# wenet-e2e/wenet

Hardware: AMD Instinct MI355X
Metric: audio-seconds/sec (RTF^-1), 12L Conformer fbank80, ctc_prefix_beam_search (higher is better)
Workload: dtype f32 (feed-forward and subsampling-conv2 GEMMs: fp32 operands as three exact bf16 planes, six plane products on the bf16 matrix cores, f32 accumulate -- error <= the v_mfma_f32 kernel's, tests/test_gpu_x6.py; everything else v_mfma_f32)

## Files before the change

include/wenet_amd.h:

```cpp
#ifndef WENET_AMD_H_
#define WENET_AMD_H_

#include <stdint.h>

#ifdef __cplusplus
extern "C" {
#endif

typedef struct wn_model wn_model;

typedef struct {
  int32_t feat_dim;
  int32_t d_model;
  int32_t n_heads;
  int32_t ffn_dim;
  int32_t n_layers;
  int32_t cnn_kernel;
  int32_t causal;
  int32_t use_dynamic_chunk;
  int32_t static_chunk_size;
  int32_t vocab;
  int32_t has_cmvn;
  int32_t dec_heads;
  int32_t dec_ffn_dim;
// ... 180 lines not shown
                    int32_t K, float alpha, int32_t act, void* stream);
int wn_op_gemm_skinny(const float* A_dev, const float* W_dev, const float* bias_dev,
                      const float* resid_dev, float* C_dev, int32_t M, int32_t N, int32_t K,
                      int32_t act, int32_t w_bf16, int32_t split_k, void* stream);
int wn_op_gemm_bf16_stored(const float* A_dev, const float* W_dev, const float* bias_dev,
                           const float* resid_dev, void* C_dev, int32_t M, int32_t N,
                           int32_t K, float alpha, int32_t act, int32_t c_bf16,
                           void* stream);
int wn_op_gemm_lowp(const void* A_dev, const void* W_dev, const void* a_scale_dev,
                    const void* w_scale_dev, const float* bias_dev,
                    const float* resid_dev, void* C_dev, void* c_scale_dev, int32_t M,
                    int32_t N, int32_t K, float alpha, int32_t act, int32_t c_mode,
                    int32_t dtype, void* stream);
int wn_op_mx_quantize(const float* x_dev, int32_t rows, int32_t K, void* q_dev,
                      void* scale_dev, void* stream);
int wn_op_ffn_fused(const float* X_dev, const float* W1_dev, const float* b1_dev,
                    const float* W2_dev, const float* b2_dev, float* x_inout_dev,
                    const float* ln_w_dev, const float* ln_b_dev, float* y_out_dev,
                    int32_t M, int32_t D, int32_t F, int32_t act, float alpha, float eps,
                    void* stream);
int wn_op_gemm_x6(const float* A_dev, const float* W_dev, const float* bias_dev,
                  const float* resid_dev, float* C_dev, int32_t M, int32_t N, int32_t K,
                  float alpha, int32_t act, int32_t bm, int32_t reps, void* stream);
int wn_op_ffn_x6(const float* X_dev, const float* W1_dev, const float* b1_dev,
                 const float* W2_dev, const float* b2_dev, float* x_inout_dev,
                 const float* ln_w_dev, const float* ln_b_dev, float* y_out_dev, int32_t M,
                 int32_t D, int32_t F, int32_t act, float alpha, float eps, int32_t reps,
                 void* stream);
int wn_op_gemm_x6r(const float* A_dev, const float* W_dev, const float* bias_dev,
                   float* x_inout_dev, const float* ln_w_dev, const float* ln_b_dev,
                   float* y_dev, float* C_dev, int32_t M, int32_t N, int32_t epi, float alpha,
                   float eps, int32_t reps, void* stream);

int wn_op_gemm_x6r512(const float* A, const float* W, const float* bias, float* x_inout,
                      const float* ln_w, const float* ln_b, float* y, const float* W2,
                      const float* bias2, float* C, int32_t M, int32_t N, int32_t epi, float alpha,
                      float eps, int32_t reps, void* stream);
int wn_op_log_add(const double* a_dev, const double* b_dev, double* out_dev,
                  int32_t n, void* stream);
int wn_op_layernorm(const float* x_dev, const float* w_dev, const float* b_dev,
                    float* y_dev, int32_t M, int32_t D, float eps, void* stream);

typedef struct wn_attention_op {
  const void* Q; const void* K; const void* V;
  int32_t ldq, ldk, ldv;
  int32_t q_rows, kv_rows;
  const float* P; int32_t ldp, p_rows;
  const int32_t* p_off;
  const float* bias_u; const float* bias_v;
  void* O; int32_t ldo;
  const int32_t* q_off; const int32_t* q_len;
  const int32_t* kv_off; const int32_t* kv_len;
  int32_t n_seq, n_heads;
  int32_t mask_mode, chunk_size, left_chunks;
  float scale;
  int32_t flags;
  int32_t precision;
  int32_t x6_galign;
} wn_attention_op;
#define WN_ATTN_FOLD 1
#define WN_ATTN_PREFOLD 2
#define WN_ATTN_QKV_BF16 4
#define WN_ATTN_O_BF16 8
int wn_op_attention(const wn_attention_op* op, int32_t* form_out, void* stream);
int wn_op_dwconv(const float* x, int32_t ldx, const float* wt, const float* bias,
                 const float* cpad, const float* ln_w, const float* ln_b, int32_t norm_mode,
// ... 58 lines not shown
```

wenet_amd/_lib.py:

```python
import ctypes
import os
from ctypes import (POINTER, Structure, c_char_p, c_double, c_float, c_int32,
                    c_int64, c_void_p)

_HERE = os.path.dirname(os.path.abspath(__file__))
LIB_PATH = os.path.join(_HERE, 'libwenet_amd.so')


class WnConfig(Structure):
    _fields_ = [(n, c_int32) for n in (
        'feat_dim', 'd_model', 'n_heads', 'ffn_dim', 'n_layers', 'cnn_kernel',
        'causal', 'use_dynamic_chunk', 'static_chunk_size', 'vocab',
        'has_cmvn', 'dec_heads', 'dec_ffn_dim', 'dec_layers', 'dec_r_layers',
        'bidirectional', 'sos', 'eos', 'max_pos')] + [('norm_eps', c_float)] + [
            (n, c_int32) for n in ('encoder_type', 'input_layer', 'activation',
                                   'key_bias', 'cnn_norm',
                                   'dec_activation', 'dec_key_bias', 'dec_src_key_bias',
                                   'dec_learned_pos', 'dec_max_pos')]


class WnTransducerConfig(Structure):
    _fields_ = [(n, c_int32) for n in ('pred_embed', 'pred_hidden', 'pred_layers', 'pred_out',
                                       'join_dim', 'blank')]


class WnTensor(Structure):
    _fields_ = [('name', c_char_p), ('data', POINTER(c_float)),
                ('numel', c_int64)]


class WnStreamResult(Structure):
    _fields_ = [('n_hyps', POINTER(c_int32)), ('hyp_lens', POINTER(c_int32)),
                ('hyp_tlens', POINTER(c_int32)), ('hyp_tokens', POINTER(c_int32)),
                ('hyp_times', POINTER(c_int32)), ('hyp_scores', POINTER(c_double)),
                ('hyp_viterbi', POINTER(c_double)), ('frames_decoded', POINTER(c_int32)),
                ('trailing_blank', POINTER(c_int32)), ('max_len', c_int32)]


class WnAttentionOp(Structure):
    _fields_ = [('Q', c_void_p), ('K', c_void_p), ('V', c_void_p),
                ('ldq', c_int32), ('ldk', c_int32), ('ldv', c_int32),
                ('q_rows', c_int32), ('kv_rows', c_int32),
                ('P', c_void_p), ('ldp', c_int32), ('p_rows', c_int32),
                ('p_off', POINTER(c_int32)), ('bias_u', c_void_p), ('bias_v', c_void_p),
                ('O', c_void_p), ('ldo', c_int32),
                ('q_off', POINTER(c_int32)), ('q_len', POINTER(c_int32)),
                ('kv_off', POINTER(c_int32)), ('kv_len', POINTER(c_int32)),
                ('n_seq', c_int32), ('n_heads', c_int32), ('mask_mode', c_int32),
                ('chunk_size', c_int32), ('left_chunks', c_int32), ('scale', c_float),
                ('flags', c_int32), ('precision', c_int32), ('x6_galign', c_int32)]


EXPORTS = [
    'wn_last_error', 'wn_version', 'wn_model_create', 'wn_model_destroy', 'wn_model_clone',
    'wn_model_set_precision', 'wn_model_get_precision', 'wn_batch_size', 'wn_model_set_encode_gate', 'wn_op_gemm_bf16',
    'wn_op_gemm_bf16_stored',
    'wn_attention_beam_search', 'wn_attention_beam_search_prompt', 'wn_attention_truncated',
    'wn_op_gemm_skinny', 'wn_encode_chunk_batch', 'wn_op_gemm_lowp', 'wn_op_mx_quantize', 'wn_op_ffn_fused', 'wn_op_gemm_x6', 'wn_op_ffn_x6', 'wn_op_gemm_x6r', 'wn_op_gemm_x6r512', 'wn_profile_kernel_name', 'wn_profile_ffn_split', 'wn_profile_ffn_clocks', 'wn_profile_gemm_clocks', 'wn_filter_blank_embedding',
    'wn_workspace_create', 'wn_resample_length', 'wn_resample', 'wn_fbank', 'wn_log_mel', 'wn_encode', 'wn_encode_chunk', 'wn_set_encoder_out',
    'wn_ctc_logprobs', 'wn_set_ctc_probs', 'wn_ctc_greedy_search', 'wn_ctc_force_align',
    'wn_set_context_graph', 'wn_ctc_prefix_beam_search', 'wn_attention_rescoring', 'wn_rescore', 'wn_rescore_prefetch', 'wn_decoder_forward', 'wn_decoder_next_topk', 'wn_op_gemm',
    'wn_op_layernorm', 'wn_op_log_add', 'wn_op_attention', 'wn_op_dwconv', 'wn_op_conv1',
    'wn_op_ctc_rows', 'wn_debug_set', 'wn_profile_enable',
    'wn_profile_collect', 'wn_tune_set', 'wn_model_tune_set', 'wn_tune_get',
    'wn_stream_create', 'wn_stream_destroy', 'wn_stream_set_endpoint', 'wn_stream_reset',
    'wn_stream_advance', 'wn_stream_advance_encoded',
    'wn_model_create_transducer', 'wn_transducer_greedy_search', 'wn_op_lstm_step',
    'wn_op_joint_argmax',
]

_lib = None


def lib():
    global _lib
    if _lib is not None:
        return _lib
    if not os.path.exists(LIB_PATH):
        raise RuntimeError(
            f'{LIB_PATH} is missing: build it with `python -m wenet_amd.build` '
            '(hipcc --offload-arch=gfx950). wenet_amd has no CPU fallback.')
    import torch
    L = ctypes.CDLL(LIB_PATH, mode=ctypes.RTLD_GLOBAL)
    i32, i64, f32, vp = c_int32, c_int64, c_float, c_void_p
    pi32, pf64 = POINTER(c_int32), POINTER(c_double)
    L.wn_last_error.restype = c_char_p
    L.wn_profile_kernel_name.restype = c_char_p
    L.wn_profile_kernel_name.argtypes = [vp]
    L.wn_profile_ffn_split.restype = c_int32
    L.wn_profile_ffn_split.argtypes = [vp]
    L.wn_profile_ffn_clocks.argtypes = [POINTER(ctypes.c_uint64)]
# ... 29 lines not shown
    L.wn_stream_create.argtypes = [vp, i32, i32, i32, i32, POINTER(vp), vp]
    L.wn_stream_destroy.argtypes = [vp]
    L.wn_stream_set_endpoint.argtypes = [vp, f32, f32]
    L.wn_stream_reset.argtypes = [vp, i32, pi32, vp]
    L.wn_stream_advance.argtypes = [vp, i32, pi32, vp, pi32, i32, i32, i32,
                                    POINTER(WnStreamResult), vp]
    L.wn_stream_advance_encoded.argtypes = [vp, i32, pi32, vp, pi32, i32, i32,
                                            POINTER(WnStreamResult), vp]
    L.wn_attention_rescoring.argtypes = [vp, i32, pi32, pi32, pi32, i32, f32,
                                         POINTER(f32), POINTER(f32), vp]
    L.wn_rescore.argtypes = [vp, i32, pi32, pi32, pi32, pf64, i32, c_double, c_double, pi32,
                             POINTER(f32), pf64, pf64, POINTER(f32), vp]
    L.wn_rescore_prefetch.argtypes = [vp, i32, vp]
    L.wn_decoder_forward.argtypes = [vp, i32, i32, i32, pi32, pi32, i32, vp, vp]
    L.wn_decoder_next_topk.argtypes = [vp, i32, pi32, pi32, pi32, i32, i32,
                                       POINTER(f32), pi32, vp]
    L.wn_attention_beam_search.argtypes = [vp, i32, i32, f32, pi32, pi32, vp]
    L.wn_attention_beam_search_prompt.argtypes = [vp, i32, i32, f32, pi32, i32, pi32, pi32, vp]
    L.wn_attention_truncated.argtypes = [vp]
    L.wn_op_gemm.argtypes = [vp, vp, vp, vp, vp, i32, i32, i32, f32, i32, vp]
    L.wn_op_gemm_skinny.argtypes = [vp, vp, vp, vp, vp, i32, i32, i32, i32, i32, i32, vp]
    L.wn_op_gemm_bf16.argtypes = L.wn_op_gemm.argtypes
    L.wn_op_gemm_bf16_stored.argtypes = [vp, vp, vp, vp, vp, i32, i32, i32, f32, i32, i32, vp]
    L.wn_op_gemm_lowp.argtypes = [vp, vp, vp, vp, vp, vp, vp, vp, i32, i32, i32, f32, i32, i32,
                                  i32, vp]
    L.wn_op_mx_quantize.argtypes = [vp, i32, i32, vp, vp, vp]
    L.wn_op_ffn_fused.argtypes = [vp, vp, vp, vp, vp, vp, vp, vp, vp, i32, i32, i32, i32, f32,
                                  f32, vp]
    L.wn_op_gemm_x6.argtypes = [vp, vp, vp, vp, vp, i32, i32, i32, f32, i32, i32, i32, vp]
    L.wn_op_ffn_x6.argtypes = [vp, vp, vp, vp, vp, vp, vp, vp, vp, i32, i32, i32, i32, f32,
                               f32, i32, vp]
    L.wn_filter_blank_embedding.argtypes = [vp, vp, pi32, pi32, vp]
    L.wn_op_gemm_x6r.argtypes = [vp, vp, vp, vp, vp, vp, vp, vp, i32, i32, i32, f32, f32, i32, vp]
    L.wn_op_gemm_x6r512.argtypes = [vp, vp, vp, vp, vp, vp, vp, vp, vp, vp, i32, i32, i32, f32, f32,
                                    i32, vp]
    L.wn_model_set_precision.argtypes = [vp, i32]
    L.wn_model_get_precision.argtypes = [vp]
    L.wn_batch_size.argtypes = [vp]
    L.wn_batch_size.restype = i32
    L.wn_model_set_encode_gate.argtypes = [vp, vp]
    L.wn_op_layernorm.argtypes = [vp, vp, vp, vp, i32, i32, f32, vp]
    L.wn_op_log_add.argtypes = [vp, vp, vp, i32, vp]
    L.wn_op_attention.argtypes = [POINTER(WnAttentionOp), pi32, vp]
    L.wn_op_dwconv.argtypes = [vp, i32, vp, vp, vp, vp, vp, i32, vp, i32, pi32, pi32, i32, i32,
                               i32, i32, i32, i32, f32, vp]
    L.wn_op_conv1.argtypes = [vp, vp, vp, vp, vp, vp, pi32, pi32, i32, i32, i32, i32, i32, i32,
                              vp]
    L.wn_op_ctc_rows.argtypes = [vp, i32, i32, i32, i32, i32, f32, vp, vp, vp, i32, vp]
    L.wn_debug_set.argtypes = [vp, c_char_p, i32]
    L.wn_tune_set.argtypes = [c_char_p, i32]
    L.wn_model_tune_set.argtypes = [vp, c_char_p, i32]
    L.wn_tune_get.argtypes = [vp, c_char_p, pi32]
    L.wn_profile_enable.argtypes = [vp, i32]
    L.wn_profile_collect.argtypes = [vp, pi32, pf64, pf64]
    L.wn_model_create_transducer.argtypes = [POINTER(WnConfig), POINTER(WnTransducerConfig),
                                             POINTER(WnTensor), i32, i32, POINTER(vp)]
    L.wn_transducer_greedy_search.argtypes = [vp, i32, pi32, pi32, i32, pi32, vp]
    L.wn_op_lstm_step.argtypes = [vp, POINTER(vp), i32, vp, vp, vp, vp, vp, vp, i32, i32, i32,
                                  i32, vp]
    L.wn_op_joint_argmax.argtypes = [vp, i32, vp, i32, pi32, pi32, vp, vp, i32, i32, i32, pi32,
                                     POINTER(f32), vp]
    for n in EXPORTS:
        if n not in ('wn_last_error', 'wn_version', 'wn_model_destroy',
                     'wn_resample_length', 'wn_profile_kernel_name',
                     'wn_profile_ffn_split'):
            getattr(L, n).restype = i32
# ... 29 lines not shown
```

wenet_amd/csrc/cabi_ops.hip:

```cpp
#include "model_state.h"
#include "x6.h"

namespace wn {
namespace {

__global__ __launch_bounds__(256) void conv1_image_unpack_kernel(
    const char* __restrict__ img, int tiles, const int* __restrict__ t1_off,
    const int* __restrict__ t1_len, int F1, int C, float* __restrict__ out) {
  const int b = blockIdx.y;
  const int n = t1_len[b] * F1 * (C / 8);
  const int ne = (F1 + 1) / 2;
  for (int i = blockIdx.x * 256 + threadIdx.x; i < n; i += gridDim.x * 256) {
    const int cg = i % (C / 8), px = i / (C / 8);
    const int fr = px / F1, pos = px - fr * F1;
    const int f1 = pos < ne ? 2 * pos : 2 * (pos - ne) + 1;
    const int row = (t1_off[b] + fr) * F1;
    const char* src = img + x3_piece(cg >> 1, tiles, row + pos, cg & 1);
    const bf16x8 p0 = *reinterpret_cast<const bf16x8*>(src);
    const bf16x8 p1 = *reinterpret_cast<const bf16x8*>(src + X3_REC);
    const bf16x8 p2 = *reinterpret_cast<const bf16x8*>(src + 2 * X3_REC);
    float* o = out + ((int64_t)row + f1) * C + cg * 8;
#pragma unroll
    for (int e = 0; e < 8; ++e) o[e] = ((float)p0[e] + (float)p1[e]) + (float)p2[e];
  }
// ... 210 lines not shown
      g1.A = X; g1.lda = D; g1.a_bytes = (int64_t)M * D * 4;
      g1.epi = 0; g1.C = hf.as<float>(); g1.ldc = F;
      g2.A = hf.as<float>(); g2.lda = F; g2.a_bytes = (int64_t)M * F * 4;
    } else {
      WN_TRY(x6_split(X, M, D, D, x3.as<char>(), s));
      g1.A3 = x3.as<char>(); g1.epi = 2; g1.C3 = h3.as<char>();
      g2.A3 = h3.as<char>();
    }
    WN_TRY(gemm_x6(g1, s));
    WN_TRY(gemm_x6(g2, s));
    if (r + 1 < reps) continue;
    WN_TRY(ffn_reduce_ln(x, part.as<float>(), S, b2, alpha, ln_w, ln_b, nullptr, nullptr, y,
                         M, D, eps, 0, s));
  }
  return 0;
}

int wn_op_gemm_x6r(const float* A, const float* W, const float* bias, float* x_inout,
                   const float* ln_w, const float* ln_b, float* y, float* C, int32_t M,
                   int32_t N, int32_t epi, float alpha, float eps, int32_t reps, void* stream) {
  WN_CHECK(A && W && M > 0 && gemm_x6r_supported(M, N, 256, epi), "gemm_x6r: shape");
  hipStream_t s = (hipStream_t)stream;
  static thread_local DevBuf w3;
  WN_TRY(w3.ensure(x6_bytes(N, 256)));
  WN_TRY(x6_split(W, N, 256, 256, w3.as<char>(), s));
  X6RArgs a;
  a.A = A; a.lda = 256; a.W3 = w3.as<char>(); a.bias = bias; a.M = M; a.N = N; a.epi = epi;
  a.C = C; a.ldc = N; a.resid = x_inout; a.ldr = N; a.alpha = alpha; a.x_out = x_inout;
  a.ldx = N; a.ln_w = ln_w; a.ln_b = ln_b; a.eps = eps; a.y = y; a.ldy = N;
  for (int r = 0; r < (reps > 0 ? reps : 1); ++r) WN_TRY(gemm_x6r(a, s));
  return 0;
}

int wn_op_gemm_x6r512(const float* A, const float* W, const float* bias, float* x_inout,
                      const float* ln_w, const float* ln_b, float* y, const float* W2,
                      const float* bias2, float* C, int32_t M, int32_t N, int32_t epi, float alpha,
                      float eps, int32_t reps, void* stream) {
  WN_CHECK(A && W && M > 0 && gemm_x6r512_supported(M, N, epi), "gemm_x6r512: shape");
  WN_CHECK(epi != 3 || (W2 && C), "gemm_x6r512: the chained epilogue needs W2 and C");
  hipStream_t s = (hipStream_t)stream;
  static thread_local DevBuf w3, w3b;
  WN_TRY(w3.ensure(x6_bytes(N, 512)));
  WN_TRY(x6_split(W, N, 512, 512, w3.as<char>(), s));
  X6RArgs a;
  a.A = A; a.lda = 512; a.K = 512; a.W3 = w3.as<char>(); a.bias = bias; a.M = M; a.N = N;
  a.epi = epi; a.C = C; a.ldc = epi == 3 ? 512 : N; a.resid = x_inout; a.ldr = N; a.alpha = alpha;
  a.x_out = x_inout; a.ldx = N; a.ln_w = ln_w; a.ln_b = ln_b; a.eps = eps; a.y = y; a.ldy = N;
  if (epi == 3) {
    WN_TRY(w3b.ensure(x6_bytes(1024, 512)));
    WN_TRY(x6_split(W2, 1024, 512, 512, w3b.as<char>(), s));
    a.W3b = w3b.as<char>(); a.bias2 = bias2;
  }
  for (int r = 0; r < (reps > 0 ? reps : 1); ++r) WN_TRY(gemm_x6r(a, s));
  return 0;
}

int wn_op_log_add(const double* a_dev, const double* b_dev, double* out_dev,
                  int32_t n, void* stream) {
  return log_add_pairs(a_dev, b_dev, out_dev, n, (hipStream_t)stream);
}

int wn_op_layernorm(const float* x, const float* w, const float* b, float* y,
                    int32_t M, int32_t D, float eps, void* stream) {
  return layernorm(x, D, w, b, y, D, M, D, eps, (hipStream_t)stream);
}

// ... 197 lines not shown
```

wenet_amd/csrc/gemm_x6r.hip:

```cpp
#include "common.h"
#include "kernels.h"
#include "rowregs.h"
#include "attn_x6_img.h"
#include "x6.h"

namespace wn {

namespace {

#define WAVE_LDS_ORDER() asm volatile("s_waitcnt lgkmcnt(0)" ::: "memory")

constexpr int RK = 256;
constexpr int RKB = RK / 16;

__device__ unsigned long long g_x6r_clk[8][8];
template <int NT, int EPI, int PF, int PRO = 0>
__global__ __launch_bounds__(256, 1) void x6r_kernel(X6RArgs p) {
  const bool stamp = blockIdx.x == gridDim.x / 2 && threadIdx.x == 0;
  unsigned long long k0 = __builtin_readcyclecounter(), k1 = 0, k2 = 0, k3 = 0, k4 = 0, kp = 0;
  const unsigned long long rt0 = __builtin_amdgcn_s_memrealtime();
  __shared__ float red[2][4][32];
  constexpr int PATCH = 4 * 32 * (NT * 128 + 16) > 32 * 1040 ? 4 * 32 * (NT * 128 + 16) : 32 * 1040;
  __shared__ __attribute__((aligned(16))) char patch[PATCH];
  __shared__ __attribute__((aligned(16))) char ximg[RKB * 3 * 1024];
  const int tid = threadIdx.x, lane = tid & 63;
  const int wave = __builtin_amdgcn_readfirstlane(tid >> 6);
  __builtin_assume(wave >= 0 && wave < 4);
  const int hi = lane >> 5, li = lane & 31;
  const int m0 = blockIdx.x * 32;
  const int row = m0 + li;
  const int rowc = min(row, p.M - 1);

  {
    f32x4 rowv[8];
    if constexpr (PRO == 1) {
      const int c = lane * 4;
      const f32x4 b2 = *reinterpret_cast<const f32x4*>(p.pro_b2 + c);
      f32x4 acc8[8], xo8[8];
      int r8[8];
#pragma unroll
      for (int j = 0; j < 8; ++j) {
        r8[j] = min(m0 + wave * 8 + j, p.M - 1);
        acc8[j] = b2;
        xo8[j] = *reinterpret_cast<const f32x4*>(p.pro_x + (int64_t)r8[j] * RK + c);
      }
      int sl = 0;
      for (; sl + 4 <= p.pro_S; sl += 4) {
        f32x4 v[4][8];
#pragma unroll
        for (int u = 0; u < 4; ++u)
#pragma unroll
          for (int j = 0; j < 8; ++j)
            v[u][j] = *reinterpret_cast<const f32x4*>(
                p.pro_P + ((int64_t)(sl + u) * p.M + r8[j]) * RK + c);
#pragma unroll
        for (int u = 0; u < 4; ++u)
#pragma unroll
// ... 151 lines not shown
        bb.load(a.ln_b, lane);
#pragma unroll
        for (int r = 0; r < R; ++r) {
          const float var = sq[r] * (1.0f / RK);
          const float rstd = 1.0f / sqrtf(var + a.eps);
#pragma unroll
          for (int e = 0; e < 4; ++e)
            acc[r].v[e] = (acc[r].v[e] - sm[r]) * rstd * ww.v[e] + bb.v[e];
        }
      } else {
        RowRegs<4> sc, sh;
        sc.load(a.ln_w, lane);
        sh.load(a.ln_b, lane);
#pragma unroll
        for (int r = 0; r < R; ++r)
#pragma unroll
          for (int e = 0; e < 4; ++e) acc[r].v[e] = fmaf(acc[r].v[e], sc.v[e], sh.v[e]);
      }
#pragma unroll
      for (int r = 0; r < R; ++r)
#pragma unroll
        for (int e = 0; e < 4; ++e) rowv[r][e] = on[r] ? silu_f(acc[r].v[e]) : 0.f;
    } else {
#pragma unroll
      for (int j = 0; j < 8; ++j) {
        const int r = min(m0 + wave * 8 + j, p.M - 1);
        rowv[j] = *reinterpret_cast<const f32x4*>(p.A + (int64_t)r * p.lda + lane * 4);
      }
    }
    asm volatile("" : "+v"(rowv[0]), "+v"(rowv[7]));
    kp = __builtin_readcyclecounter();
#pragma unroll
    for (int j = 0; j < 8; ++j)
      *reinterpret_cast<f32x4*>(patch + (wave * 8 + j) * 1040 + lane * 16) = rowv[j];
  }
  const int Tn = (p.N + 31) >> 5;
  const char* wb = reinterpret_cast<const char*>(p.W3) + ((int64_t)wave * NT * 3) * X3_REC +
                   lane * 16;
  const int64_t kstride = (int64_t)Tn * X3_TILE;
  bf16x8 wf[PF + 1][NT][3];
  auto load_w = [&](int ks) {
    const char* q = wb + ks * kstride;
#pragma unroll
    for (int t = 0; t < NT; ++t)
#pragma unroll
      for (int pl = 0; pl < 3; ++pl)
        wf[ks % (PF + 1)][t][pl] = *reinterpret_cast<const bf16x8*>(q + (t * 3 + pl) * X3_REC);
  };
  constexpr bool RELOAD = PF == 1;
  auto load_rec = [&](int ks, int t, int pl) {
    wf[ks % (PF + 1)][t][pl] =
        *reinterpret_cast<const bf16x8*>(wb + ks * kstride + (t * 3 + pl) * X3_REC);
  };
  __builtin_amdgcn_sched_barrier(0);
#pragma unroll
  for (int s = 0; s < (RELOAD ? 2 : PF); ++s) load_w(s);
  __syncthreads();
  k1 = __builtin_readcyclecounter();
  auto split_quarter = [&]() {
#pragma unroll
    for (int j = 0; j < RKB / 4; ++j) {
      const int ks = wave * (RKB / 4) + j;
      const f32x4 a4 = *reinterpret_cast<const f32x4*>(patch + li * 1040 + ks * 64 + hi * 32);
      const f32x4 b4 = *reinterpret_cast<const f32x4*>(patch + li * 1040 + ks * 64 + hi * 32 + 16);
      bf16x8 x3[3];
#pragma unroll
      for (int e = 0; e < 4; ++e) {
        const Split3 sa = split3(a4[e]), sb = split3(b4[e]);
        x3[0][e] = sa.h0; x3[1][e] = sa.h1; x3[2][e] = sa.h2;
        x3[0][4 + e] = sb.h0; x3[1][4 + e] = sb.h1; x3[2][4 + e] = sb.h2;
      }
#pragma unroll
      for (int pl = 0; pl < 3; ++pl)
        *reinterpret_cast<bf16x8*>(ximg + (ks * 3 + pl) * 1024 + lane * 16) = x3[pl];
    }
  };
  bf16x8 xf[2][3];
  auto load_x = [&](int ks) {
#pragma unroll
    for (int pl = 0; pl < 3; ++pl)
      xf[ks & 1][pl] = *reinterpret_cast<const bf16x8*>(ximg + (ks * 3 + pl) * 1024 + lane * 16);
  };
  split_quarter();
  __syncthreads();
  load_x(0);

  f32x16 acc[NT];
#pragma unroll
  for (int t = 0; t < NT; ++t)
#pragma unroll
    for (int r = 0; r < 16; ++r) acc[t][r] = 0.f;
  const int ecol = wave * NT * 32 + 4 * hi;
  f32x4 ebias[NT][4], elw[(EPI == 1 || EPI == 3) ? NT : 1][4], elb[(EPI == 1 || EPI == 3) ? NT : 1][4];
#pragma unroll
  for (int t = 0; t < NT; ++t)
#pragma unroll
    for (int g = 0; g < 4; ++g) {
// ... 5 lines not shown
        elb[t][g] = *reinterpret_cast<const f32x4*>(p.ln_b + c);
      }
    }
  k2 = __builtin_readcyclecounter();

  constexpr int PW[6] = {2, 0, 1, 1, 0, 0}, PX[6] = {0, 2, 1, 0, 1, 0};
#pragma unroll
  for (int ks = 0; ks < RKB; ++ks) {
    if (!RELOAD && ks + PF < RKB) load_w(ks + PF);
    if (ks + 1 < RKB) load_x(ks + 1);
#pragma unroll
    for (int q = 0; q < 6; ++q) {
#pragma unroll
      for (int t = 0; t < NT; ++t)
        acc[t] = __builtin_amdgcn_mfma_f32_32x32x16_bf16(wf[ks % (PF + 1)][t][PW[q]],
                                                         xf[ks & 1][PX[q]], acc[t], 0, 0, 0);
      if (RELOAD && ks + 2 < RKB && (q == 0 || q == 3 || q == 5)) {
        __builtin_amdgcn_sched_barrier(0);
#pragma unroll
        for (int t = 0; t < NT; ++t) load_rec(ks + 2, t, q == 0 ? 2 : q == 3 ? 1 : 0);
      }
    }
    __builtin_amdgcn_sched_barrier(0);
  }

  asm volatile("" : "+v"(acc[0]), "+v"(acc[NT - 1]));
  k3 = __builtin_readcyclecounter();
  const int col0 = wave * NT * 32;
  constexpr int SEG = NT * 128;
  constexpr int PST = SEG + 16;
  constexpr int LPR = SEG / 16;
  constexpr int NIT = 32 * LPR / 64;
  __syncthreads();
  char* wp = patch + wave * (32 * PST);
  auto put = [&](const f32x4 (&v)[NT][4]) {
#pragma unroll
    for (int t = 0; t < NT; ++t)
#pragma unroll
      for (int g = 0; g < 4; ++g)
        *reinterpret_cast<f32x4*>(wp + li * PST + (t * 32 + 8 * g + 4 * hi) * 4) = v[t][g];
  };
  auto get = [&](f32x4 (&v)[NT][4]) {
#pragma unroll
    for (int t = 0; t < NT; ++t)
#pragma unroll
      for (int g = 0; g < 4; ++g)
        v[t][g] = *reinterpret_cast<const f32x4*>(wp + li * PST + (t * 32 + 8 * g + 4 * hi) * 4);
  };
  auto store_rows = [&](float* base, int ld) {
#pragma unroll
    for (int it = 0; it < NIT; ++it) {
      const int q = it * 64 + lane, r = q / LPR, pc = q - r * LPR;
      const f32x4 v = *reinterpret_cast<const f32x4*>(wp + r * PST + pc * 16);
      if (m0 + r < p.M && col0 + pc * 4 < p.N)
        *reinterpret_cast<f32x4*>(base + (int64_t)(m0 + r) * ld + col0 + pc * 4) = v;
    }
  };
  if constexpr (EPI == 0) {
    f32x4 v[NT][4];
#pragma unroll
    for (int t = 0; t < NT; ++t)
#pragma unroll
      for (int g = 0; g < 4; ++g) {
        v[t][g] = f32x4{acc[t][4 * g], acc[t][4 * g + 1], acc[t][4 * g + 2], acc[t][4 * g + 3]} +
                  ebias[t][g];
      }
    put(v);
// ... 172 lines not shown
        }
    s2 += __shfl_xor(s2, 32, 64);
    if (hi == 0) red[1][wave][li] = s2;
    __syncthreads();
    const float var =
        ((red[1][0][li] + red[1][1][li]) + (red[1][2][li] + red[1][3][li])) / (float)p.N;
    const float rstd = 1.0f / sqrtf(var + p.eps);
#pragma unroll
    for (int t = 0; t < NT; ++t)
#pragma unroll
      for (int g = 0; g < 4; ++g) {
        const f32x4 w = elw[t][g], b = elb[t][g];
#pragma unroll
        for (int e = 0; e < 4; ++e) v[t][g][e] = (v[t][g][e] - mean) * rstd * w[e] + b[e];
      }
    if (p.y != nullptr) {
      put(v);
      store_rows(p.y, p.ldy);
    }
    if constexpr (EPI == 1) {
      if (p.y3 != nullptr) {
        const int tiles_m = (p.M + 31) >> 5;
#pragma unroll
        for (int t = 0; t < NT; ++t)
          x3_store_tile(v[t], p.y3, (col0 + t * 32) >> 4, tiles_m, blockIdx.x, hi, li);
      }
    }
    if constexpr (EPI == 3) {
      __syncthreads();
#pragma unroll
      for (int t = 0; t < NT; ++t)
#pragma unroll
        for (int g = 0; g < 4; ++g)
          *reinterpret_cast<f32x4*>(patch + li * 1040 + (col0 + t * 32 + 8 * g + 4 * hi) * 4) =
              v[t][g];
      constexpr int NT2 = 4, PF2 = 2;
      const char* wb2 = reinterpret_cast<const char*>(p.W3b) +
                        ((int64_t)wave * NT2 * 3) * X3_REC + lane * 16;
      const int64_t kstride2 = (int64_t)16 * X3_TILE;
      bf16x8 wf2[PF2 + 1][NT2][3];
      auto load_w2 = [&](int ks) {
        const char* q = wb2 + ks * kstride2;
#pragma unroll
        for (int t = 0; t < NT2; ++t)
#pragma unroll
          for (int pl = 0; pl < 3; ++pl)
            wf2[ks % (PF2 + 1)][t][pl] =
                *reinterpret_cast<const bf16x8*>(q + (t * 3 + pl) * X3_REC);
      };
#pragma unroll
      for (int s2i = 0; s2i < PF2; ++s2i) load_w2(s2i);
      __syncthreads();
      split_quarter();
      __syncthreads();
      load_x(0);
      f32x16 acc2[NT2];
#pragma unroll
      for (int t = 0; t < NT2; ++t)
#pragma unroll
        for (int r = 0; r < 16; ++r) acc2[t][r] = 0.f;
      f32x4 ebias2[NT2][4];
#pragma unroll
      for (int t = 0; t < NT2; ++t)
#pragma unroll
        for (int g = 0; g < 4; ++g) {
          ebias2[t][g] = f32x4{0.f, 0.f, 0.f, 0.f};
          if (p.bias2)
            ebias2[t][g] = *reinterpret_cast<const f32x4*>(p.bias2 + wave * NT2 * 32 + t * 32 +
                                                           8 * g + 4 * hi);
        }
#pragma unroll
      for (int ks = 0; ks < RKB; ++ks) {
        if (ks + PF2 < RKB) load_w2(ks + PF2);
        if (ks + 1 < RKB) load_x(ks + 1);
#pragma unroll
        for (int q = 0; q < 6; ++q)
#pragma unroll
          for (int t = 0; t < NT2; ++t)
            acc2[t] = __builtin_amdgcn_mfma_f32_32x32x16_bf16(wf2[ks % (PF2 + 1)][t][PW[q]],
                                                              xf[ks & 1][PX[q]], acc2[t], 0, 0, 0);
        __builtin_amdgcn_sched_barrier(0);
      }
      __syncthreads();
      const int c2 = wave * NT2 * 32;
      char* wp2 = patch + wave * (32 * 272);
#pragma unroll
      for (int u = 0; u < 2; ++u)
#pragma unroll
        for (int g = 0; g < 4; ++g) {
          const int c = c2 + 2 * u * 32 + 8 * g + 4 * hi;
          f32x4 a = f32x4{acc2[2 * u][4 * g], acc2[2 * u][4 * g + 1], acc2[2 * u][4 * g + 2],
                          acc2[2 * u][4 * g + 3]};
          f32x4 gt = f32x4{acc2[2 * u + 1][4 * g], acc2[2 * u + 1][4 * g + 1],
                           acc2[2 * u + 1][4 * g + 2], acc2[2 * u + 1][4 * g + 3]};
          a += ebias2[2 * u][g];
          gt += ebias2[2 * u + 1][g];
          f32x4 o;
#pragma unroll
          for (int e = 0; e < 4; ++e) o[e] = a[e] * wn_rcp(1.0f + wn_exp(-gt[e]));
          *reinterpret_cast<f32x4*>(wp2 + li * 272 + (u * 32 + 8 * g + 4 * hi) * 4) = o;
        }
#pragma unroll
      for (int it = 0; it < 8; ++it) {
        const int q = it * 64 + lane, r = q >> 4, pc = q & 15;
        const f32x4 o = *reinterpret_cast<const f32x4*>(wp2 + r * 272 + pc * 16);
        if (m0 + r < p.M)
          *reinterpret_cast<f32x4*>(p.C + (int64_t)(m0 + r) * p.ldc + c2 / 2 + pc * 4) = o;
      }
    }
  }
  asm volatile("s_waitcnt vmcnt(0)" ::: "memory");
  k4 = __builtin_readcyclecounter();
  if (stamp) {
    unsigned long long* o = g_x6r_clk[(EPI == 4 ? 0 : EPI) + (PRO != 0 ? 4 : 0)];
    o[0] = k0; o[1] = k1; o[2] = k2; o[3] = k3; o[4] = k4; o[5] = kp;
    o[6] = rt0; o[7] = __builtin_amdgcn_s_memrealtime();
  }
}

template <int NT, int EPI, int PF, int PRO = 0>
int launch_x6r(const X6RArgs& a, hipStream_t s) {
  hipLaunchKernelGGL((x6r_kernel<NT, EPI, PF, PRO>), dim3(cdiv(a.M, 32)), dim3(256), 0, s, a);
  WN_HIP(hipGetLastError());
  return 0;
}

}

int gemm_x6r_clocks(unsigned long long* out) {
  WN_HIP(hipDeviceSynchronize());
  WN_HIP(hipMemcpyFromSymbol(out, HIP_SYMBOL(g_x6r_clk), sizeof(g_x6r_clk)));
  return 0;
}

bool gemm_x6r_supported(int M, int N, int K, int epi) {
  if (K == 512) return gemm_x6r512_supported(M, N, epi);
  if (K != RK || M <= 0) return false;
  if (epi == 1 || epi == 3) return N == 256;
  if (epi == 2) return N == 512;
  if (epi == 4) return N == 768;
  return N == 256 || N == 512 || N == 768;
}

int gemm_x6r(const X6RArgs& a, hipStream_t s) {
  if (a.K == 512) return gemm_x6r512(a, s);
  WN_CHECK(a.K == RK, "gemm_x6r: K must be 256 or 512");
  if (a.pro_P) {
    WN_CHECK((a.epi == 0 || a.epi == 4) && a.N == 768 && a.W3 && a.M > 0 && a.pro_S >= 1 &&
                 a.pro_b2 && a.pro_x && a.ln_w && a.ln_b && a.C && a.ldc % 4 == 0,
             "gemm_x6r: prologue fold arguments");
    if (a.epi == 4) {
      WN_CHECK(a.at_img && a.at_P && a.at_ldp % 4 == 0 && a.at_u && a.at_v && a.at_row_utt &&
                   a.at_off && a.bias, "gemm_x6r: key-tile image arguments (epi 4)");
      return launch_x6r<6, 4, 1, 1>(a, s);
    }
    return launch_x6r<6, 0, 1, 1>(a, s);
  }
  WN_CHECK((a.A || a.dw_on) && a.W3 && a.lda % 4 == 0 && a.epi != 4 &&
               gemm_x6r_supported(a.M, a.N, RK, a.epi), "gemm_x6r: shape");
  if (a.dw_on) {
    WN_CHECK(a.epi == 1 && a.N == 256 && a.W3 && a.M > 0 && a.dw.D == 256 && a.dw.M == a.M &&
                 a.dw.x && a.dw.ldx % 4 == 0 && a.dw.wt && a.dw.bias && a.dw.cpad && a.dw.ln_w &&
                 a.dw.ln_b && a.dw.row_utt && a.dw.off && a.dw.len && a.dw.K >= 1 &&
                 a.resid && a.x_out && a.ln_w && a.ln_b && (a.y || a.y3) && a.ldr % 4 == 0 &&
                 a.ldx % 4 == 0 && a.ldy % 4 == 0, "gemm_x6r: depthwise-conv prologue arguments");
    return launch_x6r<2, 1, 3, 2>(a, s);
  }
  if (a.epi == 1) {
    WN_CHECK(a.resid && a.x_out && a.ln_w && a.ln_b && (a.y || a.y3) && a.ldr % 4 == 0 && a.ldx % 4 == 0 &&
                 a.ldy % 4 == 0, "gemm_x6r: row-LN epilogue arguments");
    return launch_x6r<2, 1, 3>(a, s);
  }
  if (a.epi == 3) {
    WN_CHECK(a.resid && a.x_out && a.ln_w && a.ln_b && a.ldr % 4 == 0 && a.ldx % 4 == 0 &&
                 (a.y == nullptr || a.ldy % 4 == 0) && a.W3b && a.C && a.ldc % 4 == 0,
             "gemm_x6r: chained row-LN + GLU arguments");
    return launch_x6r<2, 3, 3>(a, s);
  }
  WN_CHECK(a.C && a.ldc % 4 == 0, "gemm_x6r: no output");
  if (a.epi == 2) return launch_x6r<4, 2, 2>(a, s);
  switch (a.N) {
    case 256: return launch_x6r<2, 0, 3>(a, s);
    case 512: return launch_x6r<4, 0, 2>(a, s);
    default: return launch_x6r<6, 0, 1>(a, s);
  }
}

}
```

wenet_amd/csrc/tune.h:

```cpp
#pragma once
#include <stdint.h>

#include <string>

namespace wn {

#define WN_TUNE_KEYS(X)                                                                         \
                          \
  X(gemm_tile_bf16, 0)                                                                          \
                            \
  X(bf16_store, 1)                                                                              \
                      \
  X(lp_probe, 0)                                                                                \
                       \
  X(attn_split, 0)                                                                              \
                     \
  X(attn_bf16, 1)                                                                               \
                 \
  X(attn_bf16_nw, 0)                                                                            \
                                                                            \
  X(attn_bf16_defer, 80)                                                                        \
                                                              \
  X(attn_bf16_dma, 1)                                                                           \
                        \
  X(qkv_bf16, 1)                                                                                \
            \
  X(fp8_min_tiles, 192)                                                                         \
       \
  X(ffn_fused, 1)                                                                               \
                                                                   \
  X(gemm_x6, 1)                                                                                 \
                                         \
  X(x6_linear, 1)                                                                               \
                      \
  X(x6_af32, 0)                                                                                 \
            \
  X(x6_conv_af32, 0)                                                                            \
     \
  X(enc_gate_pos, 0)                                                                            \
                                                            \
  X(x6_conv_bm, 128)                                                                            \
                    \
  X(x6_probe, 0)                                                                                \
                     \
  X(ffn_x6f, 1)                                                                                 \
            \
  X(ffn_ximg, 1)                                                                                \
                             \
  X(ffn_x6f_ring, 3)                                                                            \
                  \
  X(ffn_x6f_var, 0)                                                                             \
                                                                        \
  X(x6r, 1)                                                                                     \
                  \
  X(x6r_chain, 1)                                                                               \
          \
  X(x6r_dwc, 1)                                                                                 \
        \
  X(x6r_pro, 1)                                                                                 \
            \
  X(x6r512_rows, 0)                                                                             \
                 \
  X(gemm_rowln, 1)                                                                              \
          \
  X(dwconv_tiled, 1)                                                                            \
                               \
  X(attn_x6, 1)                                                                                 \
                   \
  X(attn_xcd, 1)                                                                                \
        \
  X(attn_x6_galign, 2)                                                                          \
                             \
  X(attn_x6_order, 1)                                                                           \
    \
  X(attn_x6_var, 0)                                                                             \
        \
  X(attn_fold, 1)                                                                               \
                  \
  X(rescore_groups, 1)                                                                          \
                                                \
  X(rescore_prefetch, 1)                                                                        \
    \
  X(beam_weak_hash, 0)                                                                          \
                                                                              \
  X(beam_lds_pool, 1)                                                                           \
    \
  X(sync_spin, 1)                                                                               \
                         \
  X(ctc_wave, 1)                                                                                \
        \
// ... 23 lines not shown
```

Measured before the change: 72300.

## Fit two x6r blocks per CU by reusing the activation-image LDS for patches

For the NT=2 x6r GEMM variants, the separate patch scratch buffer is removed and its staging is carved into quarters of the ximg LDS buffer. This lets launch bounds request two blocks per CU, raising occupancy to hide memory latency. The split loads are read into registers before being overwritten, and the second GEMM's bias load is deferred into the last K iterations. A tune key (x6r_pair=0) restores single-block occupancy via dynamic LDS padding. It also adds a test entry point, wn_op_gemm_x6r_chain.

```diff
diff --git a/include/wenet_amd.h b/include/wenet_amd.h
--- a/include/wenet_amd.h
+++ b/include/wenet_amd.h
@@ -236,6 +236,11 @@
                    float* y_dev, float* C_dev, int32_t M, int32_t N, int32_t epi, float alpha,
                    float eps, int32_t reps, void* stream);
 
+int wn_op_gemm_x6r_chain(const float* A, const float* W, const float* bias, float* x_inout,
+                         const float* ln_w, const float* ln_b, float* y, const float* W2,
+                         const float* bias2, float* C, int32_t M, float alpha, float eps,
+                         void* stream);
+
 int wn_op_gemm_x6r512(const float* A, const float* W, const float* bias, float* x_inout,
                       const float* ln_w, const float* ln_b, float* y, const float* W2,
                       const float* bias2, float* C, int32_t M, int32_t N, int32_t epi, float alpha,
diff --git a/wenet_amd/_lib.py b/wenet_amd/_lib.py
--- a/wenet_amd/_lib.py
+++ b/wenet_amd/_lib.py
@@ -56,7 +56,7 @@
     'wn_model_set_precision', 'wn_model_get_precision', 'wn_batch_size', 'wn_model_set_encode_gate', 'wn_op_gemm_bf16',
     'wn_op_gemm_bf16_stored',
     'wn_attention_beam_search', 'wn_attention_beam_search_prompt', 'wn_attention_truncated',
-    'wn_op_gemm_skinny', 'wn_encode_chunk_batch', 'wn_op_gemm_lowp', 'wn_op_mx_quantize', 'wn_op_ffn_fused', 'wn_op_gemm_x6', 'wn_op_ffn_x6', 'wn_op_gemm_x6r', 'wn_op_gemm_x6r512', 'wn_profile_kernel_name', 'wn_profile_ffn_split', 'wn_profile_ffn_clocks', 'wn_profile_gemm_clocks', 'wn_filter_blank_embedding',
+    'wn_op_gemm_skinny', 'wn_encode_chunk_batch', 'wn_op_gemm_lowp', 'wn_op_mx_quantize', 'wn_op_ffn_fused', 'wn_op_gemm_x6', 'wn_op_ffn_x6', 'wn_op_gemm_x6r', 'wn_op_gemm_x6r_chain', 'wn_op_gemm_x6r512', 'wn_profile_kernel_name', 'wn_profile_ffn_split', 'wn_profile_ffn_clocks', 'wn_profile_gemm_clocks', 'wn_filter_blank_embedding',
     'wn_workspace_create', 'wn_resample_length', 'wn_resample', 'wn_fbank', 'wn_log_mel', 'wn_encode', 'wn_encode_chunk', 'wn_set_encoder_out',
     'wn_ctc_logprobs', 'wn_set_ctc_probs', 'wn_ctc_greedy_search', 'wn_ctc_force_align',
     'wn_set_context_graph', 'wn_ctc_prefix_beam_search', 'wn_attention_rescoring', 'wn_rescore', 'wn_rescore_prefetch', 'wn_decoder_forward', 'wn_decoder_next_topk', 'wn_op_gemm',
@@ -152,6 +152,7 @@
                                f32, i32, vp]
     L.wn_filter_blank_embedding.argtypes = [vp, vp, pi32, pi32, vp]
     L.wn_op_gemm_x6r.argtypes = [vp, vp, vp, vp, vp, vp, vp, vp, i32, i32, i32, f32, f32, i32, vp]
+    L.wn_op_gemm_x6r_chain.argtypes = [vp, vp, vp, vp, vp, vp, vp, vp, vp, vp, i32, f32, f32, vp]
     L.wn_op_gemm_x6r512.argtypes = [vp, vp, vp, vp, vp, vp, vp, vp, vp, vp, i32, i32, i32, f32, f32,
                                     i32, vp]
     L.wn_model_set_precision.argtypes = [vp, i32]
diff --git a/wenet_amd/csrc/cabi_ops.hip b/wenet_amd/csrc/cabi_ops.hip
--- a/wenet_amd/csrc/cabi_ops.hip
+++ b/wenet_amd/csrc/cabi_ops.hip
@@ -266,6 +266,25 @@
   return 0;
 }
 
+int wn_op_gemm_x6r_chain(const float* A, const float* W, const float* bias, float* x_inout,
+                         const float* ln_w, const float* ln_b, float* y, const float* W2,
+                         const float* bias2, float* C, int32_t M, float alpha, float eps,
+                         void* stream) {
+  WN_CHECK(A && W && W2 && C && M > 0 && gemm_x6r_supported(M, 256, 256, 3), "gemm_x6r: shape");
+  hipStream_t s = (hipStream_t)stream;
+  static thread_local DevBuf w3, w3b;
+  WN_TRY(w3.ensure(x6_bytes(256, 256)));
+  WN_TRY(x6_split(W, 256, 256, 256, w3.as<char>(), s));
+  WN_TRY(w3b.ensure(x6_bytes(512, 256)));
+  WN_TRY(x6_split(W2, 512, 256, 256, w3b.as<char>(), s));
+  X6RArgs a;
+  a.A = A; a.lda = 256; a.W3 = w3.as<char>(); a.bias = bias; a.M = M; a.N = 256; a.epi = 3;
+  a.C = C; a.ldc = 256; a.resid = x_inout; a.ldr = 256; a.alpha = alpha; a.x_out = x_inout;
+  a.ldx = 256; a.ln_w = ln_w; a.ln_b = ln_b; a.eps = eps; a.y = y; a.ldy = 256;
+  a.W3b = w3b.as<char>(); a.bias2 = bias2;
+  return gemm_x6r(a, s);
+}
+
 int wn_op_gemm_x6r512(const float* A, const float* W, const float* bias, float* x_inout,
                       const float* ln_w, const float* ln_b, float* y, const float* W2,
                       const float* bias2, float* C, int32_t M, int32_t N, int32_t epi, float alpha,
diff --git a/wenet_amd/csrc/gemm_x6r.hip b/wenet_amd/csrc/gemm_x6r.hip
--- a/wenet_amd/csrc/gemm_x6r.hip
+++ b/wenet_amd/csrc/gemm_x6r.hip
@@ -15,14 +15,20 @@
 
 __device__ unsigned long long g_x6r_clk[8][8];
 template <int NT, int EPI, int PF, int PRO = 0>
-__global__ __launch_bounds__(256, 1) void x6r_kernel(X6RArgs p) {
+__global__ __launch_bounds__(256, NT == 2 ? 2 : 1) void x6r_kernel(X6RArgs p) {
   const bool stamp = blockIdx.x == gridDim.x / 2 && threadIdx.x == 0;
   unsigned long long k0 = __builtin_readcyclecounter(), k1 = 0, k2 = 0, k3 = 0, k4 = 0, kp = 0;
   const unsigned long long rt0 = __builtin_amdgcn_s_memrealtime();
   __shared__ float red[2][4][32];
-  constexpr int PATCH = 4 * 32 * (NT * 128 + 16) > 32 * 1040 ? 4 * 32 * (NT * 128 + 16) : 32 * 1040;
+  constexpr bool PAIR = NT == 2;
+  constexpr int QUART = (RKB / 4) * 3 * 1024;
+  constexpr int QST = 272;
+  constexpr int PATCH = PAIR ? 16 :
+      4 * 32 * (NT * 128 + 16) > 32 * 1040 ? 4 * 32 * (NT * 128 + 16) : 32 * 1040;
   __shared__ __attribute__((aligned(16))) char patch[PATCH];
   __shared__ __attribute__((aligned(16))) char ximg[RKB * 3 * 1024];
+  static_assert(!PAIR || sizeof(red) + sizeof(ximg) <= 163840 / 2 - 1280, "NT = 2: LDS of two blocks per CU");
+  static_assert(!PAIR || (32 * QST <= QUART && NT * 128 + 16 == QST), "NT = 2: the patches fit their quarter");
   const int tid = threadIdx.x, lane = tid & 63;
   const int wave = __builtin_amdgcn_readfirstlane(tid >> 6);
   __builtin_assume(wave >= 0 && wave < 4);
@@ -240,7 +246,11 @@
     kp = __builtin_readcyclecounter();
 #pragma unroll
     for (int j = 0; j < 8; ++j)
-      *reinterpret_cast<f32x4*>(patch + (wave * 8 + j) * 1040 + lane * 16) = rowv[j];
+      if constexpr (PAIR)
+        *reinterpret_cast<f32x4*>(ximg + (lane >> 4) * QUART + (wave * 8 + j) * QST +
+                                  (lane & 15) * 16) = rowv[j];
+      else
+        *reinterpret_cast<f32x4*>(patch + (wave * 8 + j) * 1040 + lane * 16) = rowv[j];
   }
   const int Tn = (p.N + 31) >> 5;
   const char* wb = reinterpret_cast<const char*>(p.W3) + ((int64_t)wave * NT * 3) * X3_REC +
@@ -266,11 +276,27 @@
   __syncthreads();
   k1 = __builtin_readcyclecounter();
   auto split_quarter = [&]() {
+    f32x4 qa[PAIR ? RKB / 4 : 1], qb[PAIR ? RKB / 4 : 1];
+    if constexpr (PAIR) {
+      const char* qp = ximg + wave * QUART + li * QST + hi * 32;
+#pragma unroll
+      for (int j = 0; j < RKB / 4; ++j) {
+        qa[j] = *reinterpret_cast<const f32x4*>(qp + j * 64);
+        qb[j] = *reinterpret_cast<const f32x4*>(qp + j * 64 + 16);
+      }
+      WAVE_LDS_ORDER();
+    }
 #pragma unroll
     for (int j = 0; j < RKB / 4; ++j) {
       const int ks = wave * (RKB / 4) + j;
-      const f32x4 a4 = *reinterpret_cast<const f32x4*>(patch + li * 1040 + ks * 64 + hi * 32);
-      const f32x4 b4 = *reinterpret_cast<const f32x4*>(patch + li * 1040 + ks * 64 + hi * 32 + 16);
+      f32x4 a4, b4;
+      if constexpr (PAIR) {
+        a4 = qa[j];
+        b4 = qb[j];
+      } else {
+        a4 = *reinterpret_cast<const f32x4*>(patch + li * 1040 + ks * 64 + hi * 32);
+        b4 = *reinterpret_cast<const f32x4*>(patch + li * 1040 + ks * 64 + hi * 32 + 16);
+      }
       bf16x8 x3[3];
 #pragma unroll
       for (int e = 0; e < 4; ++e) {
@@ -342,7 +368,7 @@
   constexpr int LPR = SEG / 16;
   constexpr int NIT = 32 * LPR / 64;
   __syncthreads();
-  char* wp = patch + wave * (32 * PST);
+  char* wp = PAIR ? ximg + wave * QUART : patch + wave * (32 * PST);
   auto put = [&](const f32x4 (&v)[NT][4]) {
 #pragma unroll
     for (int t = 0; t < NT; ++t)
@@ -581,8 +607,11 @@
       for (int t = 0; t < NT; ++t)
 #pragma unroll
         for (int g = 0; g < 4; ++g)
-          *reinterpret_cast<f32x4*>(patch + li * 1040 + (col0 + t * 32 + 8 * g + 4 * hi) * 4) =
-              v[t][g];
+          if constexpr (PAIR)
+            *reinterpret_cast<f32x4*>(wp + li * QST + (t * 32 + 8 * g + 4 * hi) * 4) = v[t][g];
+          else
+            *reinterpret_cast<f32x4*>(patch + li * 1040 + (col0 + t * 32 + 8 * g + 4 * hi) * 4) =
+                v[t][g];
       constexpr int NT2 = 4, PF2 = 2;
       const char* wb2 = reinterpret_cast<const char*>(p.W3b) +
                         ((int64_t)wave * NT2 * 3) * X3_REC + lane * 16;
@@ -609,19 +638,23 @@
 #pragma unroll
         for (int r = 0; r < 16; ++r) acc2[t][r] = 0.f;
       f32x4 ebias2[NT2][4];
-#pragma unroll
-      for (int t = 0; t < NT2; ++t)
-#pragma unroll
-        for (int g = 0; g < 4; ++g) {
-          ebias2[t][g] = f32x4{0.f, 0.f, 0.f, 0.f};
-          if (p.bias2)
-            ebias2[t][g] = *reinterpret_cast<const f32x4*>(p.bias2 + wave * NT2 * 32 + t * 32 +
-                                                           8 * g + 4 * hi);
-        }
+      auto load_bias2 = [&](int t0) {
+#pragma unroll
+        for (int t = t0; t < t0 + NT2 / 2; ++t)
+#pragma unroll
+          for (int g = 0; g < 4; ++g) {
+            ebias2[t][g] = f32x4{0.f, 0.f, 0.f, 0.f};
+            if (p.bias2)
+              ebias2[t][g] = *reinterpret_cast<const f32x4*>(p.bias2 + wave * NT2 * 32 + t * 32 +
+                                                             8 * g + 4 * hi);
+          }
+      };
 #pragma unroll
       for (int ks = 0; ks < RKB; ++ks) {
         if (ks + PF2 < RKB) load_w2(ks + PF2);
         if (ks + 1 < RKB) load_x(ks + 1);
+        if (ks == RKB - 2) load_bias2(0);
+        if (ks == RKB - 1) load_bias2(NT2 / 2);
 #pragma unroll
         for (int q = 0; q < 6; ++q)
 #pragma unroll
@@ -632,7 +665,7 @@
       }
       __syncthreads();
       const int c2 = wave * NT2 * 32;
-      char* wp2 = patch + wave * (32 * 272);
+      char* wp2 = PAIR ? wp : patch + wave * (32 * 272);
 #pragma unroll
       for (int u = 0; u < 2; ++u)
 #pragma unroll
@@ -668,8 +701,11 @@
 }
 
 template <int NT, int EPI, int PF, int PRO = 0>
-int launch_x6r(const X6RArgs& a, hipStream_t s) {
-  hipLaunchKernelGGL((x6r_kernel<NT, EPI, PF, PRO>), dim3(cdiv(a.M, 32)), dim3(256), 0, s, a);
+int launch_x6r(const X6RArgs& a, hipStream_t s, bool alone = false) {
+  constexpr int LDS_ALONE = 32 * 1024;
+  const int dyn = NT == 2 && alone ? LDS_ALONE : 0;
+  if (dyn) WN_MAX_DYN_LDS((x6r_kernel<NT, EPI, PF, PRO>), LDS_ALONE);
+  hipLaunchKernelGGL((x6r_kernel<NT, EPI, PF, PRO>), dim3(cdiv(a.M, 32)), dim3(256), dyn, s, a);
   WN_HIP(hipGetLastError());
   return 0;
 }
@@ -707,29 +743,30 @@
   }
   WN_CHECK((a.A || a.dw_on) && a.W3 && a.lda % 4 == 0 && a.epi != 4 &&
                gemm_x6r_supported(a.M, a.N, RK, a.epi), "gemm_x6r: shape");
+  const bool alone = tune().x6r_pair == 0;
   if (a.dw_on) {
     WN_CHECK(a.epi == 1 && a.N == 256 && a.W3 && a.M > 0 && a.dw.D == 256 && a.dw.M == a.M &&
                  a.dw.x && a.dw.ldx % 4 == 0 && a.dw.wt && a.dw.bias && a.dw.cpad && a.dw.ln_w &&
                  a.dw.ln_b && a.dw.row_utt && a.dw.off && a.dw.len && a.dw.K >= 1 &&
                  a.resid && a.x_out && a.ln_w && a.ln_b && (a.y || a.y3) && a.ldr % 4 == 0 &&
                  a.ldx % 4 == 0 && a.ldy % 4 == 0, "gemm_x6r: depthwise-conv prologue arguments");
-    return launch_x6r<2, 1, 3, 2>(a, s);
+    return launch_x6r<2, 1, 3, 2>(a, s, alone);
   }
   if (a.epi == 1) {
     WN_CHECK(a.resid && a.x_out && a.ln_w && a.ln_b && (a.y || a.y3) && a.ldr % 4 == 0 && a.ldx % 4 == 0 &&
                  a.ldy % 4 == 0, "gemm_x6r: row-LN epilogue arguments");
-    return launch_x6r<2, 1, 3>(a, s);
+    return launch_x6r<2, 1, 3>(a, s, alone);
   }
   if (a.epi == 3) {
     WN_CHECK(a.resid && a.x_out && a.ln_w && a.ln_b && a.ldr % 4 == 0 && a.ldx % 4 == 0 &&
                  (a.y == nullptr || a.ldy % 4 == 0) && a.W3b && a.C && a.ldc % 4 == 0,
              "gemm_x6r: chained row-LN + GLU arguments");
-    return launch_x6r<2, 3, 3>(a, s);
+    return launch_x6r<2, 3, 3>(a, s, alone);
   }
   WN_CHECK(a.C && a.ldc % 4 == 0, "gemm_x6r: no output");
   if (a.epi == 2) return launch_x6r<4, 2, 2>(a, s);
   switch (a.N) {
-    case 256: return launch_x6r<2, 0, 3>(a, s);
+    case 256: return launch_x6r<2, 0, 3>(a, s, alone);
     case 512: return launch_x6r<4, 0, 2>(a, s);
     default: return launch_x6r<6, 0, 1>(a, s);
   }
diff --git a/wenet_amd/csrc/tune.h b/wenet_amd/csrc/tune.h
--- a/wenet_amd/csrc/tune.h
+++ b/wenet_amd/csrc/tune.h
@@ -56,6 +56,8 @@
   X(x6r_chain, 1)                                                                               \
           \
   X(x6r_dwc, 1)                                                                                 \
+         \
+  X(x6r_pair, 1)                                                                                \
         \
   X(x6r_pro, 1)                                                                                 \
             \
```

After: 72220, median of 3. Within noise of the previous version (-0.1%).
